# skit-ai/N-Best-ASR-Transformer

Hardware: AMD Instinct MI355X
Metric: utterances/sec fine-tune (bert-base, seq128, n_best=5) (higher is better)
Workload: dtype bf16

## Files before the change

n-best-asr-transformer_amd/csrc/encoder.hip:

```cpp
#include <algorithm>
#include <vector>

#include "common.h"

namespace {

static inline size_t al(size_t x) { return (x + 255) & ~(size_t)255; }
static inline size_t take(size_t& o, size_t bytes) { const size_t at = o; o += bytes; return at; }

struct Sizes {
  size_t esz, MH, MF, M3H, MH8, MF8, st, lse;
  int64_t M;
};

static Sizes sizes(const nbest_encoder_desc* d) {
  Sizes z;
  z.esz = d->dtype == NBEST_BF16 ? 2 : 4;
  z.M = (int64_t)d->B * d->S;
  const size_t MHe = (size_t)z.M * d->H, MFe = (size_t)z.M * d->F;
  z.MH = al(MHe * z.esz); z.MF = al(MFe * z.esz); z.M3H = al(3 * MHe * z.esz);
  z.MH8 = al(MHe); z.MF8 = al(MFe);
  z.st = al((size_t)z.M * 2 * sizeof(float));
  z.lse = al((size_t)d->B * d->heads * d->S * sizeof(float));
  return z;
// ... 251 lines not shown
  if (!d->cls_top) return NBEST_OK;
  NB_CHECK(!d->w8, NBEST_ERR_ARG, "encoder: cls_top is not supported with the fp8 forward / backward (desc.w8)");
  NB_CHECK(!d->head_gate || d->head_gate_stash, NBEST_ERR_ARG, "encoder: cls_top is not supported with head_gate (the gate runs on the "
           "full-width context) unless head_gate_stash keeps the gated rows");
  NB_CHECK(!d->base_ids && !d->alpha, NBEST_ERR_ARG, "encoder: cls_top is not supported with interpolated embeddings (base_ids / alpha)");
  NB_CHECK(!d->no_param_grad, NBEST_ERR_ARG, "encoder: cls_top is not supported with no_param_grad");
  NB_CHECK(d->S >= 2, NBEST_ERR_SHAPE, "encoder: cls_top needs S >= 2 (got %d)", d->S);
  return NBEST_OK;
}
static bool cls_layer_of(const nbest_encoder_desc* d, int l) { return d->cls_top && l == d->L - 1; }

static std::vector<uint8_t> queue_skip(const nbest_encoder_desc* d, int layer_end) {
  std::vector<uint8_t> s((size_t)4 * d->L, 0);
  if (d->wgrad_skip_host) std::copy(d->wgrad_skip_host, d->wgrad_skip_host + (size_t)4 * d->L, s.begin());
  if (d->cls_top && layer_end == d->L)
    for (int j = 1; j < 4; ++j) s[(size_t)4 * (d->L - 1) + j] = 1;
  return s;
}

struct Ptrs {
  const char* wts;
  const float* prm;
  size_t esz;
  const void* W(int64_t off) const { return wts + (size_t)off * esz; }
  const float* P(int64_t off) const { return prm + off; }
};

#define RUN(x) do { int rc__ = (x); if (rc__) return rc__; } while (0)

static nbest_gemm_args gemm_nt(int dtype, const void* A, const void* B, void* C, int64_t M, int64_t N, int64_t K) {
  nbest_gemm_args g = {};
  g.A = A; g.B = B; g.C = C; g.dtype = dtype;
  g.M = M; g.N = N; g.K = K; g.lda = K; g.ldb = K; g.ldc = N;
  return g;
}

static void use_packed(nbest_gemm_args& g, const void* arena, int64_t off) {
  if (!arena || g.dtype != NBEST_BF16 || g.trans_a || g.trans_b) return;
  g.B_packed = (const char*)arena + off * 2;
  g.b_pack_bn = nbest_pack_bn(g.N);
}
static void use_packed(nbest_gemm_fp8_args& g, const void* arena, int64_t off) {
  if (!arena) return;
  g.B_packed = (const uint8_t*)arena + off;
  g.b_pack_bn = nbest_pack_bn_fp8(g.N, g.K);
}

struct GemmPass {
  int dtype; int64_t M; nbest_stream_t stream;
  uint64_t seed;
  Ptrs W; const void* packed; bool b_kn;
  bool fp8; const void *w8, *w8_packed; const float* inv_scale; const uint32_t* amax_prev; uint32_t* amax_new;
  void* colsum_ws; size_t colsum_ws_bytes; int accumulate;
};
struct GemmOp {
  const void* A; const uint8_t* A8; int a_idx;
  int64_t w_off; int mat;
  void* C; int64_t N, K; int epilogue;
  const float* bias;
  const void* R; float drop_p; uint32_t drop_stream;
  void* U; float* colsum;
  uint8_t* C8; int c_idx;
  const void* Wm; const void* Wm_packed;
};

static int layer_gemm(const GemmPass& c, const GemmOp& o) {
  if (c.fp8) {
    nbest_gemm_fp8_args g = {};
    g.A = o.A8; g.B = (const uint8_t*)c.w8 + o.w_off; g.C = o.C; g.bias = o.bias; g.R = o.R; g.U = o.U; g.C8 = o.C8;
    g.M = c.M; g.N = o.N; g.K = o.K;
    g.lda = g.ldb = o.K; g.ldc = g.ldr = g.ldu = g.ldc8 = o.N;
    use_packed(g, c.w8_packed, o.w_off);
    g.epilogue = o.epilogue; g.out_scale = 1.f; g.out_scale_dev = c.inv_scale + o.mat;
    g.drop_p = o.drop_p; g.drop_stream = o.drop_stream; g.seed = c.seed;
    g.a_amax = c.amax_prev + o.a_idx;
    if (o.C8) {
      g.c8_amax_prev = c.amax_prev + o.c_idx;
      g.c8_amax_new = c.amax_new ? c.amax_new + (int64_t)o.c_idx * NBEST_AMAX_TENSOR_WORDS : nullptr;
    }
    g.colsum_out = o.colsum; g.colsum_accumulate = c.accumulate; g.ws = c.colsum_ws; g.ws_bytes = c.colsum_ws_bytes;
    return nbest_gemm_fp8(&g, c.stream);
  }
  nbest_gemm_args g = gemm_nt(c.dtype, o.A, o.Wm ? o.Wm : c.W.W(o.w_off), o.C, c.M, o.N, o.K);
  if (c.b_kn) { g.trans_b = 1; g.ldb = o.N; }
  g.epilogue = o.epilogue; g.bias = o.bias;
  if (o.R) { g.R = o.R; g.ldr = o.N; }
  if (o.epilogue == NBEST_EPI_BIAS_DROP_RES) { g.drop_p = o.drop_p; g.drop_stream = o.drop_stream; g.seed = c.seed; }
  if (o.epilogue == NBEST_EPI_BIAS_GELU || o.epilogue == NBEST_EPI_DGELU) { g.U = o.U; g.ldu = o.N; }
  if (o.epilogue == NBEST_EPI_DGELU) {
    g.colsum_out = o.colsum; g.colsum_accumulate = g.accumulate = c.accumulate; g.ws = c.colsum_ws; g.ws_bytes = c.colsum_ws_bytes;
  }
  if (o.Wm) use_packed(g, o.Wm_packed, 0);
  else use_packed(g, c.packed, o.w_off);
  return nbest_gemm(&g, c.stream);
}

struct LayerBufs {
  void *qkv, *ctx, *r1, *x1, *u, *hact, *r2;
  void* gctx;
  float *lse, *st1, *st2;
  uint32_t* keep;
  uint8_t *x8, *ctx8, *x18, *h8;
};

static void* stash_x(const ActLayout& a, const Sizes& z, void* act, int l) { return (char*)act + a.X + (size_t)(l - a.K) * z.MH; }

static LayerBufs stashed_layer(const nbest_encoder_desc* d, const ActLayout& a, void* act, int l) {
  char* Lb = (char*)act + a.layer0 + (size_t)(l - a.K) * a.layer_stride;
  LayerBufs b = {};
  b.qkv = Lb + a.o_qkv; b.ctx = Lb + a.o_ctx; b.lse = (float*)(Lb + a.o_lse);
  b.r1 = Lb + a.o_r1; b.st1 = (float*)(Lb + a.o_st1); b.x1 = Lb + a.o_x1;
  b.u = Lb + a.o_u; b.r2 = Lb + a.o_r2; b.st2 = (float*)(Lb + a.o_st2);
  b.hact = fp8_backward_active(d) ? nullptr : Lb + a.o_hact;
  if (a.keep_bytes && d->attn_drop > 0.f) b.keep = (uint32_t*)(Lb + a.o_keep);
  if (fp8_forward_active(d)) {
    b.x8 = (uint8_t*)(Lb + a.o_x8); b.ctx8 = (uint8_t*)(Lb + a.o_ctx8);
    b.x18 = (uint8_t*)(Lb + a.o_x18); b.h8 = (uint8_t*)(Lb + a.o_h8);
  }
  if (gate_stashed(d)) b.gctx = (char*)act + a.gctx + (size_t)(l - a.K) * a.gctx_stride;
  return b;
}

static LayerBufs frozen_layer(const nbest_encoder_desc* d, const WsLayout& w, const Sizes& z, void* ws) {
  char* W = (char*)ws;
  const bool f8 = fp8_forward_active(d);
  LayerBufs b = {};
  b.qkv = W + w.dqkv; b.ctx = W + w.dctx; b.lse = (float*)(W + w.fz_lse);
  b.r1 = W + w.dR; b.st1 = (float*)(W + w.fz_st1); b.x1 = W + w.dRd;
  b.r2 = W + w.dB1; b.st2 = (float*)(W + w.fz_st2);
  b.u = f8 ? W + w.fz_u : nullptr; b.hact = f8 ? nullptr : W + w.dBig;
  if (f8) { b.x8 = (uint8_t*)(W + w.f8); b.ctx8 = b.x8 + z.MH8; b.x18 = b.ctx8 + z.MH8; b.h8 = b.x18 + z.MH8; }
  return b;
}

struct Fwd {
  const nbest_encoder_desc* d;
  GemmPass g;
  const uint8_t* key_mask;
  bool arec;
  bool q8;
  const uint32_t* AP(int idx) const { return g.fp8 ? d->aamax_prev + idx : nullptr; }
  uint32_t* AN(int idx) const { return (g.fp8 && arec) ? d->aamax_new + (int64_t)idx * NBEST_AMAX_TENSOR_WORDS : nullptr; }
  int calib(const void* t, int64_t n, int idx) const {
    if (!arec || g.fp8) return NBEST_OK;
    return nbest_internal_amax_bf16(t, n, d->aamax_new + (int64_t)idx * NBEST_AMAX_TENSOR_WORDS, (hipStream_t)g.stream);
  }
};
// ... 17 lines not shown
  const Ptrs& P = c.g.W;
  const nbest_stream_t stream = c.g.stream;
  const int64_t M = c.g.M;
  const int H = d->H, F = d->F, dt = d->dtype, t = 4 * l;
  const uint32_t s0 = d->drop_stream_base + 1 + 4 * l;
  const int heads = pl ? pl->k : d->heads, Hk = 64 * heads;
  if (c.g.fp8 && l == 0)
    RUN(nbest_internal_cast_bf16_to_fp8(xin, b.x8, M * H, c.AP(0), c.AN(0), (hipStream_t)stream));
  GemmOp wqkv = {xin, b.x8, t + 0, o.wqkv, t + 0, b.qkv, 3 * Hk, H, NBEST_EPI_BIAS, pl ? pl->bqkv : P.P(o.bqkv)};
  if (pl) { wqkv.Wm = pl->wqkv; wqkv.Wm_packed = pl->wqkv_packed; }
  RUN(layer_gemm(c.g, wqkv));
  if (cls_probs)
    RUN(nbest_internal_attention_cls_probs(b.qkv, (int64_t)d->S * H * 3, (const char*)b.qkv + H * P.esz, 3 * H, c.key_mask, cls_probs, d->S,
                                           d->B, d->S, d->heads, 64, dt, stream));
  RUN(c.calib(xin, M * H, t + 0));
  RUN(nbest_internal_attention_fwd8(b.qkv, c.key_mask, b.ctx, b.ctx8, b.lse, d->B, d->S, heads, 64, dt, d->attn_drop, d->seed, s0 + 0,
                                    stream, b.keep, c.AP(t + 1), c.AN(t + 1)));
  RUN(c.calib(b.ctx, M * Hk, t + 1));
  const void* ctx = b.ctx;
  if (d->head_gate && !pl) {
    void* gated = b.gctx ? b.gctx : b.ctx;
    RUN(nbest_head_gate_fwd(b.ctx, H, gated, H, d->head_gate + (int64_t)l * d->heads, M, d->heads, 64, dt, stream));
    ctx = gated;
  }
  GemmOp wo = {ctx, b.ctx8, t + 1, o.wo, t + 1, b.r1, H, Hk, NBEST_EPI_BIAS_DROP_RES, P.P(o.bo)};
  wo.R = xin; wo.drop_p = d->hidden_drop; wo.drop_stream = s0 + 1;
  if (pl) { wo.Wm = pl->wo; wo.Wm_packed = pl->wo_packed; }
  RUN(layer_gemm(c.g, wo));
  RUN(nbest_internal_layernorm_fwd8(b.r1, P.P(o.ln1_g), P.P(o.ln1_b), b.x1, b.x18, b.st1, M, H, d->ln_eps, dt, stream, c.AP(t + 2), c.AN(t + 2)));
  RUN(c.calib(b.x1, M * H, t + 2));
  GemmOp w1 = {b.x1, b.x18, t + 2, o.w1, t + 2, c.q8 ? nullptr : b.hact, F, H, c.q8 ? NBEST_EPI_BIAS_GELU_Q8 : NBEST_EPI_BIAS_GELU, P.P(o.b1)};
  w1.U = b.u; w1.C8 = b.h8; w1.c_idx = t + 3;
  RUN(layer_gemm(c.g, w1));
  GemmOp w2 = {b.hact, b.h8, t + 3, o.w2, t + 3, b.r2, H, F, NBEST_EPI_BIAS_DROP_RES, P.P(o.b2)};
  w2.R = b.x1; w2.drop_p = d->hidden_drop; w2.drop_stream = s0 + 2;
  RUN(layer_gemm(c.g, w2));
  RUN(c.calib(b.hact, M * F, t + 3));
  RUN(nbest_internal_layernorm_fwd8(b.r2, P.P(o.ln2_g), P.P(o.ln2_b), xout, x8_next, b.st2, M, H, d->ln_eps, dt, stream,
                                    x8_next ? c.AP(t + 4) : nullptr, x8_next ? c.AN(t + 4) : nullptr));
  return NBEST_OK;
}

static int layer_forward_cls(const Fwd& c, int l, const void* xin, void* xout, const LayerBufs& b) {
  const nbest_encoder_desc* d = c.d;
  const nbest_layer_offsets& o = d->layers_host[l];
  const Ptrs& P = c.g.W;
  const nbest_stream_t stream = c.g.stream;
  hipStream_t st = (hipStream_t)stream;
  const int H = d->H, F = d->F, dt = d->dtype, t = 4 * l;
  const int64_t B = d->B, SH = (int64_t)d->S * H;
  const uint32_t s0 = d->drop_stream_base + 1 + 4 * l;
  const bool hdrop = d->hidden_drop > 0.f;
  void* tmp = (char*)b.r2 + (size_t)B * H * P.esz;
  const GemmOp wqkv = {xin, nullptr, t + 0, o.wqkv, t + 0, b.qkv, 3 * H, H, NBEST_EPI_BIAS, P.P(o.bqkv)};
  RUN(layer_gemm(c.g, wqkv));
  RUN(nbest_attention_cls_fwd_internal(b.qkv, SH * 3, (const char*)b.qkv + H * P.esz, 3 * H, c.key_mask, b.ctx, H, d->B, d->S, d->heads, 64, dt,
                                       stream, d->attn_drop, d->seed, s0 + 0));
  auto dense_drop_res = [&](const void* A, int64_t w_off, const float* bias, int64_t N, int64_t K, const void* R, int64_t ldr, uint32_t ds,
                            void* out) -> int {
    nbest_gemm_args g = gemm_nt(dt, A, P.W(w_off), hdrop ? tmp : out, B, N, K);
    g.bias = bias;
    if (hdrop) {
      g.epilogue = NBEST_EPI_BIAS;
      RUN(nbest_gemm(&g, stream));
      return nbest_internal_rows_drop_res(tmp, N, R, ldr, out, N, B, (int)N, d->S, dt, d->hidden_drop, d->seed, ds, st);
    }
    g.epilogue = NBEST_EPI_BIAS_DROP_RES; g.R = R; g.ldr = ldr;
    return nbest_gemm(&g, stream);
  };
  const void* ctx = b.ctx;
  if (d->head_gate) {
    void* gated = b.gctx ? b.gctx : b.ctx;
    RUN(nbest_head_gate_fwd(b.ctx, H, gated, H, d->head_gate + (int64_t)l * d->heads, B, d->heads, 64, dt, stream));
    ctx = gated;
  }
  RUN(dense_drop_res(ctx, o.wo, P.P(o.bo), H, H, xin, SH, s0 + 1, b.r1));
  RUN(nbest_internal_layernorm_fwd8(b.r1, P.P(o.ln1_g), P.P(o.ln1_b), b.x1, nullptr, b.st1, B, H, d->ln_eps, dt, stream, nullptr, nullptr));
  nbest_gemm_args g = gemm_nt(dt, b.x1, P.W(o.w1), b.hact, B, F, H);
  g.epilogue = NBEST_EPI_BIAS_GELU; g.bias = P.P(o.b1); g.U = b.u; g.ldu = F;
  RUN(nbest_gemm(&g, stream));
  RUN(dense_drop_res(b.hact, o.w2, P.P(o.b2), H, F, b.x1, H, s0 + 2, b.r2));
  RUN(nbest_internal_layernorm_fwd8(b.r2, P.P(o.ln2_g), P.P(o.ln2_b), tmp, nullptr, b.st2, B, H, d->ln_eps, dt, stream, nullptr, nullptr));
  return nbest_internal_rows_drop_res(tmp, H, nullptr, 0, xout, SH, B, H, 1, dt, 0.f, 0, 0, st);
}

}

extern "C" size_t nbest_encoder_act_bytes(const nbest_encoder_desc* d) { return d ? act_layout(d, sizes(d)).total : 0; }

extern "C" int nbest_encoder_act_view(const nbest_encoder_desc* d, void* act, int layer, void** qkv, float** lse) {
  RUN(check_desc(d));
  RUN(check_cls_top(d));
  NB_CHECK(act && qkv && lse, NBEST_ERR_ARG, "encoder_act_view: null pointer");
  NB_CHECK(0 <= layer && layer < d->L, NBEST_ERR_ARG, "encoder_act_view: layer %d outside [0, L=%d)", layer, d->L);
  const ActLayout a = act_layout(d, sizes(d));
  NB_CHECK(layer >= a.K, NBEST_ERR_ARG, "encoder_act_view: layer %d < first_trainable %d (frozen layers are not stashed)", layer, a.K);
  NB_CHECK(!cls_layer_of(d, layer), NBEST_ERR_ARG, "encoder_act_view: layer %d of a cls_top stash has no lse (its attention ran on the CLS rows only)", layer);
  const LayerBufs b = stashed_layer(d, a, act, layer);
  *qkv = b.qkv; *lse = b.lse;
  return NBEST_OK;
}
extern "C" size_t nbest_encoder_ws_bytes(const nbest_encoder_desc* d) { return d ? ws_layout(d, sizes(d), wgrad_mode(d)).total : 0; }
extern "C" int nbest_encoder_wgrad_launches_per_layer(const nbest_encoder_desc* d) {
  if (!d) return 0;
  return wgrad_launches_per_layer(wgrad_mode(d), wgrad_paired(d, fp8_backward_active(d)));
}

extern "C" int nbest_encoder_wgrad_plan(const nbest_encoder_desc* d, int layer_begin, int layer_end, int32_t* out, int cap) {
  NB_CHECK(d && d->B > 0 && d->S > 0 && d->L > 0 && d->H > 0 && d->F > 0, NBEST_ERR_ARG, "encoder_wgrad_plan: bad descriptor");
  NB_CHECK(first_trainable(d) <= layer_begin && layer_begin <= layer_end && layer_end <= d->L, NBEST_ERR_ARG, "encoder_wgrad_plan: bad layer range");
  NB_CHECK(out || cap <= 0, NBEST_ERR_ARG, "encoder_wgrad_plan: null pointer");
  RUN(check_cls_top(d));
  const WgradMode wm = wgrad_mode(d);
  std::vector<int32_t> v = {wm.mode, wm.gl + wm.sets, -1, 0};
  if (wm.sets > 0) {
    const std::vector<uint8_t> qskip = queue_skip(d, layer_end);
    const WinPlan wp = window_plan(d, layer_begin, layer_end, qskip.data(), d->no_param_grad != 0, true, wm.sets);
    v[2] = wp.peel_layer; v[3] = (int32_t)wp.launches.size();
    for (const WinLaunch& w : wp.launches) {
      v.insert(v.end(), {w.after_layer, w.tiles, w.n});
      for (int i = 0; i < w.n; ++i) v.insert(v.end(), {w.e[i].layer, w.e[i].j, w.e[i].first, w.e[i].count});
    }
  }
  if ((int)v.size() <= cap) std::copy(v.begin(), v.end(), out);
  return (int)v.size();
}

extern "C" int nbest_encoder_forward(const nbest_encoder_desc* d, const void* wts, const float* prm, const int64_t* ids,
                                     const int64_t* seg, const int64_t* pos, const uint8_t* key_mask, void* act, size_t act_bytes,
                                     void* ws, size_t ws_bytes, void** hidden_out, nbest_stream_t stream) {
  RUN(check_desc(d));
  RUN(check_cls_top(d));
  NB_CHECK(wts && prm && ids && pos && key_mask && act, NBEST_ERR_ARG, "encoder_forward: null pointer");
// ... 249 lines not shown
  const nbest_encoder_desc* d = c.d;
  const nbest_layer_offsets& o = d->layers_host[l];
  const Ptrs& P = c.P;
  const nbest_stream_t stream = c.dg.stream;
  const int64_t M = c.z.M;
  const int H = d->H, F = d->F, dt = d->dtype, t = 4 * l, accumulate = c.accumulate;
  const uint32_t s0 = d->drop_stream_base + 1 + 4 * l;
  const bool f8b = c.f8b, hdrop = c.hdrop;
  RUN(nbest_internal_layernorm_bwd8(dA, b.r2, b.st2, P.P(o.ln2_g), g.dR2, (hdrop && !f8b) ? g.dRd2 : nullptr, c.GP(o.ln2_g), c.GP(o.ln2_b),
                                    c.GP(o.b2), M, H, dt, accumulate, d->hidden_drop, d->seed, s0 + 2, c.red(0), c.w.red_bytes, stream,
                                    c.fg(g.dRd8, t + 0)));
  GemmOp dw2 = {g.dRd2, g.dRd8, t + 0, o.w2, t + 3, f8b ? nullptr : g.dBig, F, H, NBEST_EPI_DGELU};
  dw2.U = b.u; dw2.colsum = c.GP(o.b1); dw2.C8 = g.dBig8; dw2.c_idx = t + 1;
  RUN(layer_gemm(c.dg, dw2));
  if (c.rec && !f8b) RUN(nbest_internal_amax_bf16(g.dBig, M * F, c.GN(t + 1), (hipStream_t)stream));
  RUN(sched.ready(3));
  GemmOp dw1 = {g.dBig, g.dBig8, t + 1, o.w1, t + 2, g.dB1, H, F, NBEST_EPI_RES};
  dw1.R = g.dR2;
  RUN(layer_gemm(c.dg, dw1));
  RUN(sched.ready(2));
  RUN(nbest_internal_layernorm_bwd8(g.dB1, b.r1, b.st1, P.P(o.ln1_g), g.dR1, (hdrop && !f8b) ? g.dRd1 : nullptr, c.GP(o.ln1_g), c.GP(o.ln1_b),
                                    c.GP(o.bo), M, H, dt, accumulate, d->hidden_drop, d->seed, s0 + 1, c.red(2), c.w.red_bytes, stream,
                                    c.fg(g.dRd8, t + 2)));
  const GemmOp dwo = {g.dRd1, g.dRd8, t + 2, o.wo, t + 1, g.dctx, H, H, NBEST_EPI_NONE};
  RUN(layer_gemm(c.dg, dwo));
  RUN(sched.ready(1));
  if (d->head_gate)
    RUN(nbest_head_gate_bwd(b.ctx, g.dctx, d->head_gate + (int64_t)l * d->heads,
                            d->head_gate_grad ? d->head_gate_grad + (int64_t)l * d->B * d->heads : nullptr, d->B, d->S, d->heads, 64, dt, stream));
  RUN(nbest_internal_attention_bwd8(b.qkv, c.key_mask, b.ctx, g.dctx, b.lse, f8b ? nullptr : g.dqkv, c.GP(o.bqkv), accumulate, c.red(3),
                                    c.w.red_bytes, d->B, d->S, d->heads, 64, dt, d->attn_drop, d->seed, s0 + 0, stream, c.fg(g.dqkv8, t + 3),
                                    b.keep));
  if (!(d->no_input_grad && l == c.a.K)) {
    GemmOp dwqkv = {g.dqkv, g.dqkv8, t + 3, o.wqkv, t + 0, dA, H, 3 * H, NBEST_EPI_RES};
    dwqkv.R = g.dR1;
    RUN(layer_gemm(c.dg, dwqkv));
  }
  return sched.ready(0);
}

static int layer_backward_cls(const Bwd& c, int l, const LayerBufs& b, const LayerGrads& g, void* dA, WgradSched& sched) {
  const nbest_encoder_desc* d = c.d;
  const nbest_layer_offsets& o = d->layers_host[l];
  const Ptrs& P = c.P;
  const nbest_stream_t stream = c.dg.stream;
  hipStream_t st = (hipStream_t)stream;
  const int H = d->H, F = d->F, dt = d->dtype, t = 4 * l, accumulate = c.accumulate;
  const uint32_t s0 = d->drop_stream_base + 1 + 4 * l;
  const bool hdrop = c.hdrop;
  const int64_t Bn = d->B, SH = (int64_t)d->S * H;
  const size_t bh = (size_t)Bn * H * c.z.esz, half = c.w.red_bytes / 2;
  void* dAc = c.ws + c.w.dR + bh;
  GemmPass dgc = c.dg;
  dgc.M = Bn; dgc.packed = nullptr;
  RUN(nbest_internal_rows_drop_res(dA, SH, nullptr, 0, dAc, H, Bn, H, 1, dt, 0.f, 0, 0, st));
  auto ln_bwd = [&](const void* dy, const void* x, const float* stats, int64_t ln_g, int64_t ln_b, int64_t bias, void* dR, void* dRd, void* red,
                    uint32_t ds) -> int {
    RUN(nbest_internal_layernorm_bwd8(dy, x, stats, P.P(ln_g), dR, nullptr, c.G(ln_g), c.G(ln_b), hdrop ? nullptr : c.G(bias), Bn, H, dt,
                                      accumulate, 0.f, 0, 0, red, half, stream, Fp8Grad{nullptr, nullptr, nullptr}));
    if (!hdrop) return NBEST_OK;
    RUN(nbest_internal_rows_drop_res(dR, H, nullptr, 0, dRd, H, Bn, H, d->S, dt, d->hidden_drop, d->seed, ds, st));
    return nbest_colsum(dRd, c.G(bias), Bn, H, H, dt, accumulate, (char*)red + half, half, stream);
  };
  RUN(ln_bwd(dAc, b.r2, b.st2, o.ln2_g, o.ln2_b, o.b2, g.dR2, g.dRd2, c.red(0), s0 + 2));
  GemmOp dw2 = {g.dRd2, nullptr, t + 0, o.w2, t + 3, g.dBig, F, H, NBEST_EPI_DGELU};
  dw2.U = b.u; dw2.colsum = c.G(o.b1);
  RUN(layer_gemm(dgc, dw2));
  GemmOp dw1 = {g.dBig, nullptr, t + 1, o.w1, t + 2, g.dB1, H, F, NBEST_EPI_RES};
  dw1.R = g.dR2;
  RUN(layer_gemm(dgc, dw1));
  RUN(ln_bwd(g.dB1, b.r1, b.st1, o.ln1_g, o.ln1_b, o.bo, g.dR1, g.dRd1, c.red(2), s0 + 1));
  const GemmOp dwo = {g.dRd1, nullptr, t + 2, o.wo, t + 1, g.dctx, H, H, NBEST_EPI_NONE};
  RUN(layer_gemm(dgc, dwo));
  if (d->head_gate)
    RUN(nbest_head_gate_bwd(b.ctx, g.dctx, d->head_gate + (int64_t)l * d->heads, nullptr, d->B, 1, d->heads, 64, dt, stream));
  RUN(nbest_internal_attention_cls_bwd(b.qkv, c.key_mask, b.ctx, g.dctx, g.dqkv, c.G(o.bqkv), accumulate, c.red(3), c.w.red_bytes, d->B, d->S,
                                       d->heads, 64, dt, d->attn_drop, d->seed, s0 + 0, stream));
  if (!(d->no_input_grad && l == c.a.K)) {
    NB_CHECK(hipMemsetAsync(g.dctx, 0, (size_t)c.z.M * H * c.z.esz, st) == hipSuccess, NBEST_ERR_LAUNCH, "encoder_backward: memset failed");
    RUN(nbest_internal_rows_drop_res(g.dR1, H, nullptr, 0, g.dctx, SH, Bn, H, 1, dt, 0.f, 0, 0, st));
    GemmOp dwqkv = {g.dqkv, nullptr, t + 3, o.wqkv, t + 0, dA, H, 3 * H, NBEST_EPI_RES};
    dwqkv.R = g.dctx;
    RUN(layer_gemm(c.dg, dwqkv));
  }
  for (int j = 3; j >= 0; --j) RUN(sched.ready(j));
  return NBEST_OK;
}
}

extern "C" int nbest_encoder_backward(const nbest_encoder_desc* d, const void* wts, const void* wts_t, const float* prm, float* grad,
                                      const int64_t* ids, const int64_t* seg, const int64_t* pos, const uint8_t* key_mask,
                                      void* act, size_t act_bytes, void* dhidden, void* ws, size_t ws_bytes, int accumulate,
                                      int layer_begin, int layer_end, int with_embeddings, nbest_stream_t stream) {
  RUN(check_desc(d));
  RUN(check_cls_top(d));
  NB_CHECK(0 <= layer_begin && layer_begin <= layer_end && layer_end <= d->L, NBEST_ERR_ARG, "encoder_backward: bad layer range");
  const bool npg = d->no_param_grad != 0;
  NB_CHECK(!npg || (!with_embeddings && d->first_trainable == 0 && !d->no_input_grad && !d->w8), NBEST_ERR_ARG,
           "encoder_backward: no_param_grad refuses with_embeddings (%d), first_trainable > 0 (%d), no_input_grad (%d) and the fp8 "
           "forward (w8): it forms the input gradient only, of a full stash", with_embeddings, d->first_trainable, d->no_input_grad);
  NB_CHECK(!d->head_gate || npg || d->head_gate_stash, NBEST_ERR_ARG, "encoder_backward: head_gate needs no_param_grad (the attention-output weight gradient would "
           "need the gated context, which the forward keeps only with head_gate_stash)");
  NB_CHECK(wts && prm && (grad || npg) && ids && pos && key_mask && act && dhidden && ws, NBEST_ERR_ARG, "encoder_backward: null pointer");
  NB_CHECK(!with_embeddings || d->word_perm, NBEST_ERR_ARG, "encoder_backward: desc.word_perm (stable argsort of this pass's ids) is required");
  NB_CHECK(layer_begin >= d->first_trainable, NBEST_ERR_ARG, "encoder_backward: layer_begin %d < first_trainable %d (those layers are not stashed)",
           layer_begin, d->first_trainable);
  NB_CHECK(!with_embeddings || (d->first_trainable == 0 && !d->no_input_grad), NBEST_ERR_ARG,
           "encoder_backward: with_embeddings needs first_trainable == 0 and no_input_grad == 0");
  const Sizes z = sizes(d);
  const ActLayout a = act_layout(d, z);
  const WgradMode wm = wgrad_mode(d);
  const WsLayout w = ws_layout(d, z, wm);
  NB_CHECK(act_bytes >= a.total, NBEST_ERR_WORKSPACE, "encoder_backward: activation stash too small");
  NB_CHECK(ws_bytes >= w.total, NBEST_ERR_WORKSPACE, "encoder_backward: workspace too small (%zu < %zu)", ws_bytes, w.total);
  const Bwd c = make_bwd(d, wts, wts_t, prm, grad, key_mask, act, ws, z, a, w, accumulate, stream);
  WgradSched sched(c, wm, layer_begin, layer_end);
  void* dA = dhidden;

  struct BatchGuard { ~BatchGuard() { nbest_internal_rowred_batch_abort(); } } batch_guard;
  for (int l = layer_end - 1; l >= layer_begin; --l) {
    const LayerBufs b = stashed_layer(d, a, act, l);
    const bool cls = cls_layer_of(d, l);
    const LayerGrads g = layer_grads(c, sched.set_of(l), cls);
    sched.begin(l, b, g);
    if (!npg) nbest_internal_rowred_batch_begin();
    RUN(cls ? layer_backward_cls(c, l, b, g, dA, sched) : layer_backward(c, l, b, g, dA, sched));
    RUN(sched.layer_end());
    if (!npg) RUN(nbest_internal_rowred_batch_flush((hipStream_t)stream));
  }
  if (!with_embeddings) return NBEST_OK;
  hipStream_t st = (hipStream_t)stream;
  const Ptrs& P = c.P;
  const int H = d->H;
  if (!accumulate) {
    hipError_t e = hipMemsetAsync(c.G(d->off_word), 0, (size_t)d->vocab * H * sizeof(float), st);
    if (e == hipSuccess) e = hipMemsetAsync(c.G(d->off_pos), 0, (size_t)d->max_pos * H * sizeof(float), st);
// ... 243 lines not shown
```

n-best-asr-transformer_amd/csrc/internal.h:

```cpp
#pragma once
#include <hip/hip_runtime_api.h>
#include <stddef.h>
#include <stdint.h>

#include "../../include/nbest_hip.h"

struct Fp8Grad;

void nbest_set_error(const char* fmt, ...);

int nbest_internal_layernorm_fwd8(const void* x, const float* gamma, const float* beta, void* y, void* y8, float* stats,
                                  int64_t M, int H, float eps, int dtype, nbest_stream_t stream, const uint32_t* a_prev, uint32_t* a_new);
int nbest_internal_layernorm_bwd8(const void* dy, const void* x, const float* stats, const float* gamma, void* dx,
                                  void* dx_drop, float* dgamma, float* dbeta, float* dbias, int64_t M, int H, int dtype,
                                  int accumulate, float drop_p, uint64_t seed, uint32_t drop_stream, void* ws,
                                  size_t ws_bytes, nbest_stream_t stream, Fp8Grad f8);
int nbest_internal_partial_rows_sum(const float* part, int nrows, int N, float* out, int accumulate, hipStream_t st);
int nbest_internal_rows_drop_res(const void* x, int64_t ldx, const void* R, int64_t ldr, void* y, int64_t ldy, int64_t rows, int N,
                                 int64_t row_mul, int dtype, float drop_p, uint64_t seed, uint32_t drop_stream, hipStream_t st);
void nbest_internal_rowred_batch_begin();
void nbest_internal_rowred_batch_abort();
int nbest_internal_rowred_batch_flush(hipStream_t st);

int nbest_internal_attention_fwd8(const void* qkv, const uint8_t* key_mask, void* ctx, void* ctx8, float* lse, int B, int S, int heads,
                                  int d, int dtype, float drop_p, uint64_t seed, uint32_t drop_stream, nbest_stream_t stream,
                                  uint32_t* keep, const uint32_t* a_prev, uint32_t* a_new);
int nbest_internal_attention_bwd8(const void* qkv, const uint8_t* key_mask, const void* ctx, const void* dctx, const float* lse,
                                  void* dqkv, float* dbias, int accumulate, void* ws, size_t ws_bytes, int B, int S, int heads,
                                  int d, int dtype, float drop_p, uint64_t seed, uint32_t drop_stream, nbest_stream_t stream, Fp8Grad f8,
                                  const uint32_t* keep);
size_t nbest_internal_attention_keep_bytes(int B, int S, int heads);
int nbest_attention_cls_fwd_internal(const void* q, int64_t ldq, const void* kv, int64_t ldkv, const uint8_t* key_mask, void* ctx,
                                     int64_t ldctx, int B, int S, int heads, int d, int dtype, nbest_stream_t stream, float drop_p,
                                     uint64_t seed, uint32_t drop_stream);
int nbest_internal_attention_cls_bwd(const void* qkv, const uint8_t* key_mask, const void* ctx, const void* dctx, void* dqkv, float* dbias,
                                     int accumulate, void* ws, size_t ws_bytes, int B, int S, int heads, int d, int dtype, float drop_p,
                                     uint64_t seed, uint32_t drop_stream, nbest_stream_t stream);
int nbest_internal_attention_cls_probs(const void* q, int64_t ldq, const void* kv, int64_t ldkv, const uint8_t* key_mask, float* probs,
                                       int64_t ldp, int B, int S, int heads, int d, int dtype, nbest_stream_t stream);

int nbest_internal_mask_to_f32(const uint8_t* mask, float* out, int64_t n, hipStream_t stream);
int nbest_internal_token_kept_row(const int32_t* origin, int32_t* out, int B, int S, int k, hipStream_t stream);

void nb_splitk_plan(int64_t tiles, int64_t K, int64_t slots, int64_t min_blocks, int* splits, int64_t* k_per_split);
int nbest_internal_splitk_reduce(const float* slab, float* C, int64_t M, int64_t N, int64_t ldc, int splits, int accumulate,
                                 float* C2, int64_t m_split, int64_t ldc2, hipStream_t st);

int nbest_gemm_f32_resolve(const nbest_gemm_args* a, nbest_gemm_plan_info* out);
int nbest_gemm_bf16_resolve(const nbest_gemm_args* a, nbest_gemm_plan_info* out);
int nbest_gemm_bf16_v2_resolve(const nbest_gemm_args* a, nbest_gemm_plan_info* out);
int nbest_gemm_f32(const nbest_gemm_args* a, hipStream_t st);
size_t nbest_gemm_bf16_ws_bytes(const nbest_gemm_args* a);
int nbest_gemm_bf16(const nbest_gemm_args* a, hipStream_t st);
size_t nbest_gemm_bf16_v2_ws_bytes(const nbest_gemm_args* a);
int nbest_gemm_bf16_v2(const nbest_gemm_args* a, hipStream_t st);
bool nbest_gemm_bf16_v2_wins(const nbest_gemm_args* a);
size_t nbest_wgrad_pair_bf16_ws_bytes(const nbest_gemm_args* a, const nbest_gemm_args* b);
int nbest_wgrad_pair_bf16(const nbest_gemm_args* a, const nbest_gemm_args* b, hipStream_t st);
int nbest_wgrad_group_bf16(const nbest_gemm_args* problems, int n, hipStream_t st);
int nbest_wgrad_window_bf16(const nbest_gemm_args* problems, const int32_t* tile_first, const int32_t* tile_count, int n, hipStream_t st);
int nbest_pack_bn_internal(int64_t N);
int nbest_pack_weights_bf16(const void* src, void* dst, const nbest_matrix_desc* descs, int n_matrices, int n_stages, hipStream_t st);

int nbest_internal_amax_bf16(const void* x, int64_t n, uint32_t* out, hipStream_t st);
int nbest_internal_cast_bf16_to_fp8(const void* src, void* dst, int64_t n, const uint32_t* a_prev, uint32_t* a_new, hipStream_t st);
```

Baseline: 13520.

## Add split-K small-M GEMM kernel for CLS-only top layer and split Q projection

Adds a bf16 GEMM kernel for small M (at most 512 rows) that splits K across 8 waves and reduces the partial sums through LDS, with fused bias/GELU/dropout/residual epilogues. In the CLS-only final layer, the forward pass now computes Q only for the CLS rows (strided over the sequence) while K/V are still computed for all tokens. The backward pass likewise splits the input-gradient GEMM into a Q part over the CLS rows and a K/V part. The aim is to avoid full-M work and badly occupied tiles for GEMMs with tiny M. The cost is an extra kernel launch and added complexity around strides and packing.

```diff
diff --git a/n-best-asr-transformer_amd/csrc/encoder.hip b/n-best-asr-transformer_amd/csrc/encoder.hip
--- a/n-best-asr-transformer_amd/csrc/encoder.hip
+++ b/n-best-asr-transformer_amd/csrc/encoder.hip
@@ -327,6 +327,7 @@
   Ptrs W; const void* packed; bool b_kn;
   bool fp8; const void *w8, *w8_packed; const float* inv_scale; const uint32_t* amax_prev; uint32_t* amax_new;
   void* colsum_ws; size_t colsum_ws_bytes; int accumulate;
+  bool rows;
 };
 struct GemmOp {
   const void* A; const uint8_t* A8; int a_idx;
@@ -337,7 +338,12 @@
   void* U; float* colsum;
   uint8_t* C8; int c_idx;
   const void* Wm; const void* Wm_packed;
-};
+  int64_t lda, ldb, ldc;
+};
+
+static int rows_gemm(const nbest_gemm_args& g, nbest_stream_t stream) {
+  return nbest_internal_gemm_rows_takes(&g) ? nbest_internal_gemm_rows(&g, stream) : nbest_gemm(&g, stream);
+}
 
 static int layer_gemm(const GemmPass& c, const GemmOp& o) {
   if (c.fp8) {
@@ -358,6 +364,9 @@
   }
   nbest_gemm_args g = gemm_nt(c.dtype, o.A, o.Wm ? o.Wm : c.W.W(o.w_off), o.C, c.M, o.N, o.K);
   if (c.b_kn) { g.trans_b = 1; g.ldb = o.N; }
+  if (o.lda) g.lda = o.lda;
+  if (o.ldb) g.ldb = o.ldb;
+  if (o.ldc) g.ldc = o.ldc;
   g.epilogue = o.epilogue; g.bias = o.bias;
   if (o.R) { g.R = o.R; g.ldr = o.N; }
   if (o.epilogue == NBEST_EPI_BIAS_DROP_RES) { g.drop_p = o.drop_p; g.drop_stream = o.drop_stream; g.seed = c.seed; }
@@ -367,7 +376,7 @@
   }
   if (o.Wm) use_packed(g, o.Wm_packed, 0);
   else use_packed(g, c.packed, o.w_off);
-  return nbest_gemm(&g, c.stream);
+  return c.rows ? rows_gemm(g, c.stream) : nbest_gemm(&g, c.stream);
 }
 
 struct LayerBufs {
@@ -491,8 +500,14 @@
   const uint32_t s0 = d->drop_stream_base + 1 + 4 * l;
   const bool hdrop = d->hidden_drop > 0.f;
   void* tmp = (char*)b.r2 + (size_t)B * H * P.esz;
-  const GemmOp wqkv = {xin, nullptr, t + 0, o.wqkv, t + 0, b.qkv, 3 * H, H, NBEST_EPI_BIAS, P.P(o.bqkv)};
-  RUN(layer_gemm(c.g, wqkv));
+  GemmOp wkv = {xin, nullptr, t + 0, o.wqkv, t + 0, (char*)b.qkv + (size_t)H * P.esz, 2 * H, H, NBEST_EPI_BIAS, P.P(o.bqkv) + H};
+  wkv.Wm = P.W(o.wqkv + (int64_t)H * H); wkv.ldc = 3 * H;
+  const int pbn = nbest_pack_bn(3 * H);
+  if (c.g.packed && pbn > 0 && H % pbn == 0 && nbest_pack_bn(2 * H) == pbn) wkv.Wm_packed = (const char*)c.g.packed + (o.wqkv + (int64_t)H * H) * 2;
+  RUN(layer_gemm(c.g, wkv));
+  nbest_gemm_args gq = gemm_nt(dt, xin, P.W(o.wqkv), b.qkv, B, H, H);
+  gq.lda = SH; gq.ldc = 3 * SH; gq.epilogue = NBEST_EPI_BIAS; gq.bias = P.P(o.bqkv);
+  RUN(rows_gemm(gq, stream));
   RUN(nbest_attention_cls_fwd_internal(b.qkv, SH * 3, (const char*)b.qkv + H * P.esz, 3 * H, c.key_mask, b.ctx, H, d->B, d->S, d->heads, 64, dt,
                                        stream, d->attn_drop, d->seed, s0 + 0));
   auto dense_drop_res = [&](const void* A, int64_t w_off, const float* bias, int64_t N, int64_t K, const void* R, int64_t ldr, uint32_t ds,
@@ -501,11 +516,11 @@
     g.bias = bias;
     if (hdrop) {
       g.epilogue = NBEST_EPI_BIAS;
-      RUN(nbest_gemm(&g, stream));
+      RUN(rows_gemm(g, stream));
       return nbest_internal_rows_drop_res(tmp, N, R, ldr, out, N, B, (int)N, d->S, dt, d->hidden_drop, d->seed, ds, st);
     }
     g.epilogue = NBEST_EPI_BIAS_DROP_RES; g.R = R; g.ldr = ldr;
-    return nbest_gemm(&g, stream);
+    return rows_gemm(g, stream);
   };
   const void* ctx = b.ctx;
   if (d->head_gate) {
@@ -517,7 +532,7 @@
   RUN(nbest_internal_layernorm_fwd8(b.r1, P.P(o.ln1_g), P.P(o.ln1_b), b.x1, nullptr, b.st1, B, H, d->ln_eps, dt, stream, nullptr, nullptr));
   nbest_gemm_args g = gemm_nt(dt, b.x1, P.W(o.w1), b.hact, B, F, H);
   g.epilogue = NBEST_EPI_BIAS_GELU; g.bias = P.P(o.b1); g.U = b.u; g.ldu = F;
-  RUN(nbest_gemm(&g, stream));
+  RUN(rows_gemm(g, stream));
   RUN(dense_drop_res(b.hact, o.w2, P.P(o.b2), H, F, b.x1, H, s0 + 2, b.r2));
   RUN(nbest_internal_layernorm_fwd8(b.r2, P.P(o.ln2_g), P.P(o.ln2_b), tmp, nullptr, b.st2, B, H, d->ln_eps, dt, stream, nullptr, nullptr));
   return nbest_internal_rows_drop_res(tmp, H, nullptr, 0, xout, SH, B, H, 1, dt, 0.f, 0, 0, st);
@@ -873,7 +888,7 @@
   const size_t bh = (size_t)Bn * H * c.z.esz, half = c.w.red_bytes / 2;
   void* dAc = c.ws + c.w.dR + bh;
   GemmPass dgc = c.dg;
-  dgc.M = Bn; dgc.packed = nullptr;
+  dgc.M = Bn; dgc.packed = nullptr; dgc.rows = true;
   RUN(nbest_internal_rows_drop_res(dA, SH, nullptr, 0, dAc, H, Bn, H, 1, dt, 0.f, 0, 0, st));
   auto ln_bwd = [&](const void* dy, const void* x, const float* stats, int64_t ln_g, int64_t ln_b, int64_t bias, void* dR, void* dRd, void* red,
                     uint32_t ds) -> int {
@@ -898,11 +913,16 @@
   RUN(nbest_internal_attention_cls_bwd(b.qkv, c.key_mask, b.ctx, g.dctx, g.dqkv, c.G(o.bqkv), accumulate, c.red(3), c.w.red_bytes, d->B, d->S,
                                        d->heads, 64, dt, d->attn_drop, d->seed, s0 + 0, stream));
   if (!(d->no_input_grad && l == c.a.K)) {
+    const bool kn = c.dg.b_kn;
+    void* tq = dAc;
+    GemmOp dwq = {g.dqkv, nullptr, t + 3, o.wqkv, t + 0, tq, H, H, NBEST_EPI_RES};
+    dwq.R = g.dR1; dwq.lda = 3 * SH; dwq.Wm = c.dg.W.W(o.wqkv); dwq.ldb = kn ? 0 : 3 * H;
+    RUN(layer_gemm(dgc, dwq));
     NB_CHECK(hipMemsetAsync(g.dctx, 0, (size_t)c.z.M * H * c.z.esz, st) == hipSuccess, NBEST_ERR_LAUNCH, "encoder_backward: memset failed");
-    RUN(nbest_internal_rows_drop_res(g.dR1, H, nullptr, 0, g.dctx, SH, Bn, H, 1, dt, 0.f, 0, 0, st));
-    GemmOp dwqkv = {g.dqkv, nullptr, t + 3, o.wqkv, t + 0, dA, H, 3 * H, NBEST_EPI_RES};
-    dwqkv.R = g.dctx;
-    RUN(layer_gemm(c.dg, dwqkv));
+    RUN(nbest_internal_rows_drop_res(tq, H, nullptr, 0, g.dctx, SH, Bn, H, 1, dt, 0.f, 0, 0, st));
+    GemmOp dwkv = {(const char*)g.dqkv + (size_t)H * c.z.esz, nullptr, t + 3, o.wqkv, t + 0, dA, H, 2 * H, NBEST_EPI_RES};
+    dwkv.R = g.dctx; dwkv.lda = 3 * H; dwkv.Wm = c.dg.W.W(o.wqkv + (kn ? (int64_t)H * H : (int64_t)H)); dwkv.ldb = kn ? 0 : 3 * H;
+    RUN(layer_gemm(c.dg, dwkv));
   }
   for (int j = 3; j >= 0; --j) RUN(sched.ready(j));
   return NBEST_OK;
diff --git a/n-best-asr-transformer_amd/csrc/gemm_rows.hip b/n-best-asr-transformer_amd/csrc/gemm_rows.hip
--- /dev/null
+++ b/n-best-asr-transformer_amd/csrc/gemm_rows.hip
@@ -0,0 +1,260 @@
+#include "common.h"
+
+namespace {
+
+constexpr int BM = 32, BN = 64, BK = 32, kWaves = 8, kThreads = kWaves * 64;
+constexpr int kUnroll = 6;
+constexpr int kRegion = BM * BN * 4;
+constexpr int kLdsBytes = kWaves * kRegion;
+constexpr int kPitchT = BN + 8;
+constexpr uint32_t kOob = 0x80000000u;
+
+struct RowsP {
+  const bf16* A; const bf16* B; bf16* C; const float* bias; const bf16* R; uint8_t* U; float* colpart;
+  int64_t M, N, K, lda, ldb, ldc, ldr, ldu;
+  int tiles_m;
+  uint32_t a_bytes, b_bytes;
+  DropCfg drop;
+};
+
+__device__ __forceinline__ bf16x8 as_frag(u32x4 v) { return __builtin_bit_cast(bf16x8, v); }
+
+template <bool TB, int EPI>
+__global__ __launch_bounds__(kThreads) void gemm_rows_kernel(RowsP p) {
+  extern __shared__ __attribute__((aligned(16))) char lds[];
+  const int tid = threadIdx.x, lane = tid & 63, wave = tid >> 6, i16 = lane & 15, g = lane >> 4;
+  const int id = xcd_remap(blockIdx.x, gridDim.x);
+  const int tile_n = id / p.tiles_m, tile_m = id - tile_n * p.tiles_m;
+  const int64_t m0 = (int64_t)tile_m * BM, n0 = (int64_t)tile_n * BN;
+
+  const __amdgpu_buffer_rsrc_t rsA = __builtin_amdgcn_make_buffer_rsrc((void*)p.A, 0, p.a_bytes, 0x00020000);
+  const __amdgpu_buffer_rsrc_t rsB = __builtin_amdgcn_make_buffer_rsrc((void*)p.B, 0, p.b_bytes, 0x00020000);
+
+  constexpr bool kHasBias = (EPI == NBEST_EPI_BIAS || EPI == NBEST_EPI_BIAS_GELU || EPI == NBEST_EPI_BIAS_DROP_RES);
+  constexpr bool kHasR = (EPI == NBEST_EPI_BIAS_DROP_RES || EPI == NBEST_EPI_RES);
+  const int erow = tid >> 4, ecq = tid & 15;
+  const int64_t em = m0 + erow, en = n0 + 4 * ecq;
+  const bool evalid = em < p.M;
+  f32x4 pb = {0, 0, 0, 0};
+  bf16x4 pr = {0, 0, 0, 0};
+  uint32_t pu = 0;
+  if (kHasBias) pb = *(const f32x4*)(p.bias + en);
+  if (kHasR && evalid) pr = *(const bf16x4*)(p.R + em * p.ldr + en);
+  if (EPI == NBEST_EPI_DGELU && evalid) pu = *(const uint32_t*)(p.U + em * p.ldu + en);
+
+  const int nk = (int)(p.K / BK), spw = (nk + kWaves - 1) / kWaves;
+  const int sbeg = wave * spw, send = (sbeg + spw < nk) ? sbeg + spw : nk;
+
+  f32x4 acc[2][4];
+#pragma unroll
+  for (int i = 0; i < 2; ++i)
+#pragma unroll
+    for (int j = 0; j < 4; ++j) acc[i][j] = f32x4{0, 0, 0, 0};
+
+  uint32_t aoff[2];
+#pragma unroll
+  for (int i = 0; i < 2; ++i) {
+    const int64_t m = m0 + 16 * i + i16;
+    aoff[i] = (m < p.M) ? (uint32_t)((m * p.lda + 8 * g) * 2) : kOob;
+  }
+  if (!TB) {
+    uint32_t boff[4];
+#pragma unroll
+    for (int j = 0; j < 4; ++j) boff[j] = (uint32_t)(((n0 + 16 * j + i16) * p.ldb + 8 * g) * 2);
+    for (int s = sbeg; s < send; s += kUnroll) {
+      u32x4 af[kUnroll][2], bfr[kUnroll][4];
+#pragma unroll
+      for (int u = 0; u < kUnroll; ++u) {
+        const bool ok = s + u < send;
+        const uint32_t ko = (uint32_t)(s + u) * (BK * 2);
+#pragma unroll
+        for (int i = 0; i < 2; ++i) af[u][i] = __builtin_amdgcn_raw_buffer_load_b128(rsA, (ok && aoff[i] != kOob) ? aoff[i] + ko : kOob, 0, 0);
+#pragma unroll
+        for (int j = 0; j < 4; ++j) bfr[u][j] = __builtin_amdgcn_raw_buffer_load_b128(rsB, ok ? boff[j] + ko : kOob, 0, 0);
+      }
+#pragma unroll
+      for (int u = 0; u < kUnroll; ++u)
+#pragma unroll
+        for (int i = 0; i < 2; ++i)
+#pragma unroll
+          for (int j = 0; j < 4; ++j)
+            acc[i][j] = __builtin_amdgcn_mfma_f32_16x16x32_bf16(as_frag(bfr[u][j]), as_frag(af[u][i]), acc[i][j], 0, 0, 0);
+    }
+  } else {
+    bf16* stg = (bf16*)(lds + wave * kRegion);
+    for (int s = sbeg; s < send; ++s) {
+      const uint32_t ko = (uint32_t)s * (BK * 2);
+      u32x4 af[2], raw[4];
+#pragma unroll
+      for (int i = 0; i < 2; ++i) af[i] = __builtin_amdgcn_raw_buffer_load_b128(rsA, aoff[i] != kOob ? aoff[i] + ko : kOob, 0, 0);
+#pragma unroll
+      for (int it = 0; it < 4; ++it) {
+        const int c = it * 64 + lane, kr = c >> 3, c8 = c & 7;
+        raw[it] = __builtin_amdgcn_raw_buffer_load_b128(rsB, (uint32_t)((((int64_t)s * BK + kr) * p.ldb + n0 + c8 * 8) * 2), 0, 0);
+      }
+#pragma unroll
+      for (int it = 0; it < 4; ++it) {
+        const int c = it * 64 + lane, kr = c >> 3, c8 = c & 7;
+        *(u32x4*)(stg + kr * kPitchT + c8 * 8) = raw[it];
+      }
+      asm volatile("s_waitcnt lgkmcnt(0)" ::: "memory");
+      __builtin_amdgcn_wave_barrier();
+      bf16x8 bfr[4];
+#pragma unroll
+      for (int j = 0; j < 4; ++j)
+#pragma unroll
+        for (int e = 0; e < 8; ++e) bfr[j][e] = stg[(8 * g + e) * kPitchT + 16 * j + i16];
+      asm volatile("s_waitcnt lgkmcnt(0)" ::: "memory");
+      __builtin_amdgcn_wave_barrier();
+#pragma unroll
+      for (int i = 0; i < 2; ++i)
+#pragma unroll
+        for (int j = 0; j < 4; ++j)
+          acc[i][j] = __builtin_amdgcn_mfma_f32_16x16x32_bf16(bfr[j], as_frag(af[i]), acc[i][j], 0, 0, 0);
+    }
+  }
+
+  float* mine = (float*)(lds + wave * kRegion);
+#pragma unroll
+  for (int i = 0; i < 2; ++i) {
+    const int row = i * 16 + i16;
+#pragma unroll
+    for (int j = 0; j < 4; ++j) {
+      const int c = j * 4 + g;
+      *(f32x4*)(mine + row * BN + ((c ^ (row & 15)) << 2)) = acc[i][j];
+    }
+  }
+  __syncthreads();
+  const int eslot = erow * BN + ((ecq ^ (erow & 15)) << 2);
+  f32x4 s4 = *(const f32x4*)((const float*)lds + eslot);
+#pragma unroll
+  for (int w = 1; w < kWaves; ++w) s4 += *(const f32x4*)((const float*)(lds + w * kRegion) + eslot);
+
+  float v[4] = {s4[0], s4[1], s4[2], s4[3]};
+  if (kHasBias) {
+#pragma unroll
+    for (int e = 0; e < 4; ++e) v[e] += pb[e];
+  }
+  if (EPI == NBEST_EPI_BIAS_GELU) {
+    float gp[4];
+#pragma unroll
+    for (int e = 0; e < 4; e += 2) {
+      f32x2 h2, g2;
+      gelu_pair_fast(f32x2{v[e], v[e + 1]}, h2, g2);
+      gp[e] = g2[0]; gp[e + 1] = g2[1]; v[e] = h2[0]; v[e + 1] = h2[1];
+    }
+    if (p.U && evalid) *(uint32_t*)(p.U + em * p.ldu + en) = gd_pack4(gp);
+  }
+  if (EPI == NBEST_EPI_BIAS_DROP_RES) {
+    if (p.drop.thr16) {
+      const uint32_t k = nb_keep4(p.drop, (uint32_t)(em * p.N + en));
+#pragma unroll
+      for (int e = 0; e < 4; ++e) v[e] = (k >> e & 1) ? v[e] * p.drop.scale : 0.f;
+    }
+  }
+  if (kHasR) {
+#pragma unroll
+    for (int e = 0; e < 4; ++e) v[e] += (float)pr[e];
+  }
+  if (EPI == NBEST_EPI_DGELU) {
+    float gd[4];
+    gd_unpack4(pu, gd);
+#pragma unroll
+    for (int e = 0; e < 4; ++e) v[e] *= gd[e];
+  }
+  if (evalid) {
+    bf16x4 o;
+#pragma unroll
+    for (int e = 0; e < 4; ++e) o[e] = (bf16)v[e];
+    st_stream((bf16x4*)(p.C + em * p.ldc + en), o, true);
+  }
+  if (EPI == NBEST_EPI_DGELU && p.colpart) {
+    __syncthreads();
+    float* cs = (float*)lds;
+    *(f32x4*)(cs + erow * BN + 4 * ecq) = evalid ? f32x4{v[0], v[1], v[2], v[3]} : f32x4{0, 0, 0, 0};
+    __syncthreads();
+    if (tid < BN) {
+      float s = 0.f;
+#pragma unroll
+      for (int r = 0; r < BM; ++r) s += cs[r * BN + tid];
+      p.colpart[(int64_t)tile_m * p.N + n0 + tid] = s;
+    }
+  }
+}
+
+template <bool TB>
+int launch_epi(const RowsP& p, int epi, int grid, hipStream_t st) {
+#define L(E)                                                                                                                      \
+  case E:                                                                                                                         \
+    (void)hipFuncSetAttribute((const void*)gemm_rows_kernel<TB, E>, hipFuncAttributeMaxDynamicSharedMemorySize, kLdsBytes);       \
+    gemm_rows_kernel<TB, E><<<grid, kThreads, kLdsBytes, st>>>(p);                                                                \
+    break;
+  switch (epi) {
+    L(NBEST_EPI_NONE) L(NBEST_EPI_BIAS) L(NBEST_EPI_BIAS_GELU) L(NBEST_EPI_BIAS_DROP_RES) L(NBEST_EPI_DGELU) L(NBEST_EPI_RES)
+    default:
+      nbest_set_error("gemm_rows: bad epilogue %d", epi);
+      return NBEST_ERR_ARG;
+  }
+#undef L
+  NB_LAUNCH_CHECK();
+  return NBEST_OK;
+}
+
+int64_t operand_bytes(int64_t rows, int64_t cols, int64_t ld) { return ((rows - 1) * ld + cols) * 2; }
+
+}
+
+bool nbest_internal_gemm_rows_takes(const nbest_gemm_args* a) {
+  if (!a || a->dtype != NBEST_BF16 || a->trans_a || a->M <= 0 || a->M > 512 || a->N <= 0 || a->N % BN || a->K <= 0 || a->K % BK) return false;
+  if (a->epilogue < NBEST_EPI_NONE || a->epilogue > NBEST_EPI_RES) return false;
+  if (a->colsum_out && a->epilogue != NBEST_EPI_DGELU) return false;
+  const int64_t ab = operand_bytes(a->M, a->K, a->lda);
+  const int64_t bb = a->trans_b ? operand_bytes(a->K, a->N, a->ldb) : operand_bytes(a->N, a->K, a->ldb);
+  return ab < (int64_t)kOob && bb < (int64_t)kOob;
+}
+
+size_t nbest_internal_gemm_rows_ws_bytes(const nbest_gemm_args* a) {
+  return (a && a->colsum_out) ? (size_t)((a->M + BM - 1) / BM) * a->N * sizeof(float) : 0;
+}
+
+extern "C" int nbest_internal_gemm_rows(const nbest_gemm_args* a, nbest_stream_t stream) {
+  NB_CHECK(a && a->A && a->B && a->C, NBEST_ERR_ARG, "gemm_rows: null pointer");
+  NB_CHECK(a->M > 0 && a->N > 0 && a->K > 0, NBEST_ERR_SHAPE, "gemm_rows: bad shape %lld x %lld x %lld", (long long)a->M, (long long)a->N,
+           (long long)a->K);
+  NB_CHECK(a->dtype == NBEST_BF16, NBEST_ERR_DTYPE, "gemm_rows: bf16 operands only (dtype %d)", a->dtype);
+  NB_CHECK(!a->trans_a, NBEST_ERR_ARG, "gemm_rows: trans_a is not built");
+  NB_CHECK(a->M <= 512, NBEST_ERR_SHAPE, "gemm_rows: M=%lld > 512", (long long)a->M);
+  NB_CHECK(a->N % BN == 0, NBEST_ERR_SHAPE, "gemm_rows: N=%lld must be a multiple of %d", (long long)a->N, BN);
+  NB_CHECK(a->K % BK == 0, NBEST_ERR_SHAPE, "gemm_rows: K=%lld must be a multiple of %d", (long long)a->K, BK);
+  NB_CHECK(a->lda % 8 == 0 && a->ldb % 8 == 0 && a->ldc % 8 == 0, NBEST_ERR_ALIGN, "gemm_rows: leading dimensions must be multiples of 8");
+  NB_CHECK(a->lda >= a->K && a->ldb >= (a->trans_b ? a->N : a->K) && a->ldc >= a->N, NBEST_ERR_SHAPE, "gemm_rows: a leading dimension is shorter than its row");
+  NB_CHECK(((uintptr_t)a->A & 15) == 0 && ((uintptr_t)a->B & 15) == 0 && ((uintptr_t)a->C & 15) == 0, NBEST_ERR_ALIGN,
+           "gemm_rows: pointers must be 16-byte aligned");
+  const int epi = a->epilogue;
+  NB_CHECK(epi >= NBEST_EPI_NONE && epi <= NBEST_EPI_RES, NBEST_ERR_ARG, "gemm_rows: epilogue %d is not built", epi);
+  if (epi == NBEST_EPI_BIAS || epi == NBEST_EPI_BIAS_GELU || epi == NBEST_EPI_BIAS_DROP_RES)
+    NB_CHECK(a->bias && ((uintptr_t)a->bias & 15) == 0, NBEST_ERR_ARG, "gemm_rows: epilogue %d needs bias", epi);
+  if (epi == NBEST_EPI_BIAS_DROP_RES || epi == NBEST_EPI_RES)
+    NB_CHECK(a->R && a->ldr % 8 == 0 && a->ldr >= a->N && ((uintptr_t)a->R & 15) == 0, NBEST_ERR_ARG, "gemm_rows: epilogue %d needs R", epi);
+  if ((epi == NBEST_EPI_BIAS_GELU && a->U) || epi == NBEST_EPI_DGELU)
+    NB_CHECK(a->U && a->ldu % 8 == 0 && a->ldu >= a->N && ((uintptr_t)a->U & 15) == 0, NBEST_ERR_ARG, "gemm_rows: epilogue %d needs U", epi);
+  NB_CHECK(!a->colsum_out || epi == NBEST_EPI_DGELU, NBEST_ERR_ARG, "gemm_rows: column sums are fused into the x GELU' epilogue only");
+  NB_CHECK(!a->colsum_out || (a->ws && a->ws_bytes >= nbest_internal_gemm_rows_ws_bytes(a)), NBEST_ERR_WORKSPACE,
+           "gemm_rows: column-sum workspace too small");
+  const int64_t ab = operand_bytes(a->M, a->K, a->lda);
+  const int64_t bb = a->trans_b ? operand_bytes(a->K, a->N, a->ldb) : operand_bytes(a->N, a->K, a->ldb);
+  NB_CHECK(ab < (int64_t)kOob && bb < (int64_t)kOob, NBEST_ERR_SHAPE, "gemm_rows: operand larger than 2 GiB");
+
+  RowsP p;
+  p.A = (const bf16*)a->A; p.B = (const bf16*)a->B; p.C = (bf16*)a->C; p.bias = a->bias; p.R = (const bf16*)a->R; p.U = (uint8_t*)a->U;
+  p.colpart = a->colsum_out ? (float*)a->ws : nullptr;
+  p.M = a->M; p.N = a->N; p.K = a->K; p.lda = a->lda; p.ldb = a->ldb; p.ldc = a->ldc; p.ldr = a->ldr; p.ldu = a->ldu;
+  p.tiles_m = (int)((a->M + BM - 1) / BM);
+  p.a_bytes = (uint32_t)ab; p.b_bytes = (uint32_t)bb;
+  p.drop = make_drop(epi == NBEST_EPI_BIAS_DROP_RES ? a->drop_p : 0.f, a->seed, a->drop_stream);
+  const int grid = p.tiles_m * (int)(a->N / BN);
+  hipStream_t st = (hipStream_t)stream;
+  if (int rc = a->trans_b ? launch_epi<true>(p, epi, grid, st) : launch_epi<false>(p, epi, grid, st)) return rc;
+  if (p.colpart) return nbest_internal_partial_rows_sum(p.colpart, p.tiles_m, (int)a->N, a->colsum_out, a->colsum_accumulate, st);
+  return NBEST_OK;
+}
diff --git a/n-best-asr-transformer_amd/csrc/internal.h b/n-best-asr-transformer_amd/csrc/internal.h
--- a/n-best-asr-transformer_amd/csrc/internal.h
+++ b/n-best-asr-transformer_amd/csrc/internal.h
@@ -62,5 +62,9 @@
 int nbest_pack_bn_internal(int64_t N);
 int nbest_pack_weights_bf16(const void* src, void* dst, const nbest_matrix_desc* descs, int n_matrices, int n_stages, hipStream_t st);
 
+bool nbest_internal_gemm_rows_takes(const nbest_gemm_args* a);
+size_t nbest_internal_gemm_rows_ws_bytes(const nbest_gemm_args* a);
+extern "C" int nbest_internal_gemm_rows(const nbest_gemm_args* a, nbest_stream_t stream);
+
 int nbest_internal_amax_bf16(const void* x, int64_t n, uint32_t* out, hipStream_t st);
 int nbest_internal_cast_bf16_to_fp8(const void* src, void* dst, int64_t n, const uint32_t* a_prev, uint32_t* a_new, hipStream_t st);
```

After: 13600 (median of 6 runs). About the same (+0.6%).
